# OPPO-Mente-Lab/PEA-Diffusion

Hardware: AMD Instinct MI355X
Metric: training images/sec (SDXL 1024px bf16, adapter-only bwd) (higher is better)
Workload: dtype bf16

## Files before the change

include/pea_hip.h:

```cpp
#ifndef PEA_HIP_H
#define PEA_HIP_H
#include <stdint.h>
#ifdef __cplusplus
extern "C" {
#endif

#define PEA_OK 0
#define PEA_E_INVALID (-1)
#define PEA_E_HIP (-2)
#define PEA_E_SHAPE (-3)
#define PEA_E_STATE (-4)
#define PEA_E_NOTFOUND (-5)
#define PEA_E_TIMEOUT (-6)

const char* pea_last_error(void);
int pea_version(void);
int pea_device_count(void);


int pea_op_gemm(const void* A, int lda, const void* W, int ldw, void* C, int ldc, int M, int N, int K, float alpha,
                const float* bias, const void* rowvec, int ldrv, int rows_per_batch, int act, void* preact,
                int ldpre, const void* res, int ldres, int out_f32, int accum_f32, void* stream);

int pea_op_gemm_qscale(const void* A, int lda, const void* W, int ldw, void* C, int ldc, int M, int N, int K, const float* bias,
                       int qscale_cols, float qscale, void* stream);

int pea_op_gemm_geglu(const void* A, int lda, const void* W, int ldw, const float* bias, void* y, void* stash, int M, int N,
                      int K, int stash_grad, int stash_rows, void* stream);

int pea_op_gemm_geglu_bwd(const void* A, int lda, const void* W, int ldw, const void* pre, int ldpre, void* C, int ldc,
                          int M, int N, int K, int form, void* stream);

int pea_op_ln_linear(const void* x, const float* gamma, const float* beta, const void* W, const float* bias, void* y,
                     void* geglu_y, int M, int N, int K, float eps, void* Wf, float* svec, float* tvec, float* stats,
                     void* stream);

int pea_op_conv3x3(const void* x, const void* w, void* y, int B, int Hs, int Ws, int Cin, int Cout, int stride,
                   int upsample2x, int transposed2, const float* bias, const void* rowvec, int ldrv,
                   const void* res, void* stream);
int pea_op_pack_conv(const float* w, void* out, int Co, int Ci, int dgrad, void* stream);
int pea_op_pack_conv_subpixel(const float* w, void* out, int Co, int Ci, int dgrad, void* stream);
int pea_op_concat2(const void* a, int C1, const void* b, int C2, void* y, long long rows, int aH, int aW, void* stream);
int pea_op_split2(const void* dy, int C1, int C2, void* da, int accum_a, void* db, int accum_b, long long rows, int aH,
                  int aW, void* stream);
long long pea_op_freeu_scratch_bytes(int B, int H, int W, int C2);
int pea_op_freeu_coef(const void* skip, int B, int H, int W, int C2, float* coef, void* scratch, void* stream);
int pea_op_concat2_freeu(const void* a, int C1, const void* b, int C2, const float* coef, void* y, int B, int H, int W, float s,
                         float bscale, int aH, int aW, void* stream);
int pea_op_upconv_subpixel(const void* x, const void* w, void* y, int B, int Hs, int Ws, int Cin, int Cout,
                           const float* bias, void* stream);
int pea_op_upconv_subpixel_dgrad(const void* dy, const void* wt, void* dx, int B, int Hs, int Ws, int Cin, int Cout,
                                 const void* res, void* stream);
int pea_op_conv_in(const float* x_nchw, const float* w, const float* bias, void* y_nhwc, int B, int Cin, int H,
                   int W, int Cout, void* stream);
int pea_op_conv_in_gather(const float* latents, const float* mask, const float* masked_latents, const float* w,
                          const float* bias, void* y_nhwc, int B, int C, int latent_batch, int cond_batch, int H, int W,
                          int Cout, void* stream);
int pea_op_conv_out(const void* x_nhwc, const float* w_packed, const float* bias, float* y_nchw, int B, int Cin,
                    int H, int W, int Cout, void* stream);
int pea_op_conv_out_dgrad(const float* dy_nchw, const float* w_packed, void* dx_nhwc, int B, int Cin, int H, int W,
                          int Cout, void* stream);
int pea_op_pack_conv_out(const float* w, float* out, int Co, int Ci, void* stream);

long long pea_op_groupnorm_scratch_bytes(int B, int HW, int C, int groups);
int pea_op_groupnorm_fwd(const void* x, const float* gamma, const float* beta, void* y, float* stats, void* scratch,
                         int B, int HW, int C, int groups, float eps, int silu, void* stream);
int pea_op_groupnorm_bwd(const void* x, const void* dy, const float* gamma, const float* beta, const float* stats,
                         void* dx, void* scratch, int B, int HW, int C, int groups, int silu, int accum,
                         void* stream);
int pea_op_layernorm_fwd(const void* x, const float* gamma, const float* beta, void* y, float* stats, int R, int C,
                         float eps, void* stream);
int pea_op_layernorm_fwd_f32(const float* x, const float* gamma, const float* beta, float* y, int R, int C, float eps,
                             void* stream);
int pea_op_layernorm_bwd(const void* x, const void* dy, const float* gamma, const float* stats, void* dx,
                         float* dgamma, float* dbeta, int R, int C, int accum, void* stream);

int pea_op_attention_fwd(const void* Q, int ldq, const void* K, int ldk, const void* V, int ldv, void* O, int ldo,
// ... 322 lines not shown
```

pea_diffusion_amd/csrc/api_ops.hip:

```cpp
#include <stdarg.h>
#include <string.h>

#include "../../include/pea_hip.h"
#include "pea_kernels.h"

static thread_local char g_err[512] = "";
void pea_set_error(const char* fmt, ...) {
  va_list ap;
  va_start(ap, fmt);
  vsnprintf(g_err, sizeof(g_err), fmt, ap);
  va_end(ap);
}

static bf16* g_zero_page = nullptr;
int pea_zero_page(const bf16** out) {
  if (!g_zero_page) {
    HIPCHK(hipMalloc((void**)&g_zero_page, 256));
    HIPCHK(hipMemset(g_zero_page, 0, 256));
  }
  *out = g_zero_page;
  return PEA_OK;
}

static AttnP attn_operands(const void* Q, int ldq, const void* K, int ldk, const void* V, int ldv, const void* O, int ldo,
// ... 25 lines not shown

extern "C" {

const char* pea_last_error(void) { return g_err; }
int pea_version(void) { return 100; }
int pea_device_count(void) {
  int n = 0;
  if (hipGetDeviceCount(&n) != hipSuccess) return 0;
  return n;
}

int pea_op_gemm(const void* A, int lda, const void* W, int ldw, void* C, int ldc, int M, int N, int K, float alpha,
                const float* bias, const void* rowvec, int ldrv, int rows_per_batch, int act, void* preact,
                int ldpre, const void* res, int ldres, int out_f32, int accum_f32, void* stream) {
  GemmP p;
  memset(&p, 0, sizeof(p));
  p.mode = 0;
  p.A = (const bf16*)A; p.lda = lda; p.W = (const bf16*)W; p.ldw = ldw; p.C = C; p.ldc = ldc;
  p.M = M; p.N = N; p.K = K; p.alpha = alpha; p.bias = bias;
  p.rowvec = (const bf16*)rowvec; p.ldrv = ldrv; p.rows_per_batch = rows_per_batch > 0 ? rows_per_batch : 1;
  p.act = act; p.preact = (bf16*)preact; p.ldpre = ldpre; p.res = (const bf16*)res; p.ldres = ldres;
  p.out_f32 = out_f32; p.accum_f32 = accum_f32;
  return launch_gemm(p, (hipStream_t)stream);
}

int pea_op_gemm_qscale(const void* A, int lda, const void* W, int ldw, void* C, int ldc, int M, int N, int K, const float* bias,
                       int qscale_cols, float qscale, void* stream) {
  GemmP p;
  memset(&p, 0, sizeof(p));
  p.A = (const bf16*)A; p.lda = lda; p.W = (const bf16*)W; p.ldw = ldw; p.C = C; p.ldc = ldc;
  p.M = M; p.N = N; p.K = K; p.alpha = 1.f; p.bias = bias; p.rows_per_batch = 1;
  p.qscale_cols = qscale_cols; p.qscale = qscale;
  return launch_gemm(p, (hipStream_t)stream);
}

int pea_op_gemm_geglu_bwd(const void* A, int lda, const void* W, int ldw, const void* pre, int ldpre, void* C, int ldc,
                          int M, int N, int K, int form, void* stream) {
  GemmP p;
  memset(&p, 0, sizeof(p));
  p.A = (const bf16*)A; p.lda = lda; p.W = (const bf16*)W; p.ldw = ldw; p.C = C; p.ldc = ldc;
  p.M = M; p.N = N; p.K = K; p.alpha = 1.f; p.rows_per_batch = 1;
  p.gbwd_pre = (const bf16*)pre; p.ldgp = ldpre; p.gbwd_form = form;
  return launch_gemm(p, (hipStream_t)stream);
}

int pea_op_gemm_geglu(const void* A, int lda, const void* W, int ldw, const float* bias, void* y, void* stash, int M, int N,
// ... 85 lines not shown
long long pea_op_freeu_scratch_bytes(int B, int H, int W, int C2) { return (long long)freeu_scratch_bytes(B, H, W, C2); }
int pea_op_freeu_coef(const void* skip, int B, int H, int W, int C2, float* coef, void* scratch, void* stream) {
  return launch_freeu_coef((const bf16*)skip, B, H, W, C2, coef, (float*)scratch, (hipStream_t)stream);
}
int pea_op_concat2_freeu(const void* a, int C1, const void* b, int C2, const float* coef, void* y, int B, int H, int W, float s,
                         float bscale, int aH, int aW, void* stream) {
  return launch_concat2_freeu((const bf16*)a, C1, (const bf16*)b, C2, coef, (bf16*)y, B, H, W, s, bscale, (hipStream_t)stream, aH, aW);
}
int pea_op_pack_conv_subpixel(const float* w, void* out, int Co, int Ci, int dgrad, void* stream) {
  return launch_pack_conv_subpix(w, (bf16*)out, Co, Ci, dgrad, (hipStream_t)stream);
}

int pea_op_pack_conv(const float* w, void* out, int Co, int Ci, int dgrad, void* stream) {
  return dgrad ? launch_pack_conv_dgrad(w, (bf16*)out, Co, Ci, (hipStream_t)stream)
               : launch_pack_conv_fwd(w, (bf16*)out, Co, Ci, (hipStream_t)stream);
}
int pea_op_pack_conv_out(const float* w, float* out, int Co, int Ci, void* stream) {
  return launch_pack_conv_out(w, out, Co, Ci, (hipStream_t)stream);
}
int pea_op_conv_in(const float* x, const float* w, const float* bias, void* y, int B, int Cin, int H, int W,
                   int Cout, void* stream) {
  return launch_conv_in(x, w, bias, (bf16*)y, B, Cin, H, W, Cout, (hipStream_t)stream);
}
int pea_op_conv_in_gather(const float* latents, const float* mask, const float* masked_latents, const float* w,
                          const float* bias, void* y, int B, int C, int latent_batch, int cond_batch, int H, int W, int Cout,
                          void* stream) {
  if (!w || !bias || !y) { pea_set_error("pea_op_conv_in_gather: null pointer"); return PEA_E_INVALID; }
  return launch_conv_in_gather(latents, mask, masked_latents, w, bias, (bf16*)y, B, C, latent_batch, cond_batch, H, W, Cout,
                               (hipStream_t)stream);
}
int pea_op_conv_out(const void* x, const float* w, const float* bias, float* y, int B, int Cin, int H, int W,
                    int Cout, void* stream) {
  return launch_conv_out((const bf16*)x, w, bias, y, B, Cin, H, W, Cout, (hipStream_t)stream);
}
int pea_op_conv_out_dgrad(const float* dy, const float* w, void* dx, int B, int Cin, int H, int W, int Cout,
                          void* stream) {
  return launch_conv_out_dgrad(dy, w, (bf16*)dx, B, Cin, H, W, Cout, (hipStream_t)stream);
}

int pea_op_groupnorm_fwd(const void* x, const float* gamma, const float* beta, void* y, float* stats, void* scratch,
                         int B, int HW, int C, int groups, float eps, int silu, void* stream) {
  return launch_groupnorm_fwd((const bf16*)x, gamma, beta, (bf16*)y, stats, (double*)scratch, B, HW, C, groups, eps,
                              silu, (hipStream_t)stream);
}
int pea_op_groupnorm_bwd(const void* x, const void* dy, const float* gamma, const float* beta, const float* stats,
                         void* dx, void* scratch, int B, int HW, int C, int groups, int silu, int accum,
// ... 247 lines not shown
```

pea_diffusion_amd/csrc/gemm.hip:

```cpp
#include <stdint.h>
#include <stdlib.h>

#include <type_traits>

#include "pea_kernels.h"

#define BK 64
constexpr int GEMM_ILV_M = 1;
constexpr int GEMM_ILV_HEAD = 4;

__device__ __forceinline__ int swz_off(int row, int chunk) { return row * 128 + ((chunk ^ ((row >> 1) & 7)) << 4); }

#ifdef PEA_GEMM_PROBES
#define PEA_PROBE(bit) (p.debug & (bit))
#else
#define PEA_PROBE(bit) false
#endif

template <int N>
__device__ __forceinline__ void wait_vmcnt() {
  static_assert(N >= 0 && N < 64, "vmcnt is a 6-bit counter");
  asm volatile("s_waitcnt vmcnt(%0)" ::"n"(N) : "memory");
}

// ... 1590 lines not shown
             "gemm: the folded-LayerNorm epilogue needs the batched-load epilogue (bf16 output, no activation / residual)");
  }
  int rc = PEA_OK;
  switch (d.inst) {
#define X(id, fn, cg, rf, gen, ...) \
    case GEMM_V##id: rc = p.mode == 0 ? fn<0, __VA_ARGS__>(p, stream) : fn<1, __VA_ARGS__>(p, stream); break;
    GEMM_TABLE(X)
#undef X
    case GEMM_GBWD_256: rc = launch_lcp<0, 256, 160, 4, 2, 4, 3, 0, 0, 3>(p, stream); break;
    case GEMM_GBWD_128: rc = launch_lcp<0, 128, 160, 4, 2, 4, 3, 0, 0, 3>(p, stream); break;
    case GEMM_GBWD_64: rc = launch_lcp<0, 64, 160, 2, 2, 4, 4, 0, 0, 3>(p, stream); break;
    case GEMM_LNF_256: rc = launch_lcp<0, 256, 160, 4, 2, 4, 3, 0, 0, 2>(p, stream); break;
    case GEMM_LNF_LC256: rc = launch_lc<0, 256, 160, 4, 2, 4, 3, false, true, 1, true>(p, stream); break;
    case GEMM_LNF_128: rc = launch_lcp<0, 128, 160, 4, 2, 4, 3, 0, 0, 2>(p, stream); break;
    case GEMM_LNF_64: rc = launch_lcp<0, 64, 160, 2, 2, 4, 4, 0, 0, 2>(p, stream); break;
    case GEMM_LNF_LC128: rc = launch_lc<0, 128, 160, 4, 2, 4, 3, false, true, 1, true>(p, stream); break;
  }
  PROF_END(stream);
  if (rc != PEA_OK) return rc;
  HIPCHK(hipGetLastError());
  return PEA_OK;
}

__global__ __launch_bounds__(256) void conv_in_kernel(const float* __restrict__ x, const float* __restrict__ w,
                                                      const float* __restrict__ bias, bf16* __restrict__ y, int B,
                                                      int Cin, int H, int W, int Cout, int pix_per_block, int ldy,
                                                      int silu) {
  extern __shared__ __attribute__((aligned(16))) char cism[];
  float* wl = (float*)cism;
  const int K = Cin * 9;
  for (int i = threadIdx.x; i < K * Cout; i += blockDim.x) {
    const int co = i / K, k = i - co * K;
    wl[k * Cout + co] = w[i];
  }
  __syncthreads();
  const int nchunk = Cout / 8;
  const int ppb = blockDim.x / nchunk;
  const int ck = threadIdx.x % nchunk, pl = threadIdx.x / nchunk;
  if (pl >= ppb) return;
  const int c0 = ck * 8;
  float bs[8];
#pragma unroll
  for (int j = 0; j < 8; ++j) bs[j] = bias[c0 + j];
  const long long npix = (long long)B * H * W;
  const long long p0 = (long long)blockIdx.x * pix_per_block;
  const long long p1 = p0 + pix_per_block < npix ? p0 + pix_per_block : npix;
// ... 11 lines not shown
          const int ix = xw + kx - 1;
          const bool ok = (unsigned)iy < (unsigned)H && (unsigned)ix < (unsigned)W;
          const float v = ok ? x[(((long long)b * Cin + ci) * H + iy) * W + ix] : 0.f;
          const float* wr = wl + (ci * 9 + ky * 3 + kx) * Cout + c0;
          const f32x4 w0 = *(const f32x4*)wr, w1 = *(const f32x4*)(wr + 4);
#pragma unroll
          for (int j = 0; j < 4; ++j) {
            acc[j] += v * w0[j];
            acc[4 + j] += v * w1[j];
          }
        }
      }
    bf16x8 o;
#pragma unroll
    for (int j = 0; j < 8; ++j) o[j] = (bf16)(silu ? siluf_(acc[j]) : acc[j]);
    *(bf16x8*)(y + pix * ldy + c0) = o;
  }
}

struct ConvGatherSrc {
  const float* lat; const float* mask; const float* masked;
  int C, lat_b, cond_b;
};
template <bool FLIP, bool GATHER = false>
__global__ __launch_bounds__(256) void conv_few4_kernel(const float* __restrict__ x, const float* __restrict__ w,
                                                        const float* __restrict__ bias, bf16* __restrict__ y, int B,
                                                        int Cs, int H, int W, int N, int groups_per_block, int ldy,
                                                        int silu, ConvGatherSrc gs) {
  extern __shared__ __attribute__((aligned(16))) char cfsm[];
  float* wl = (float*)cfsm;
  const int K = Cs * 9;
  for (int i = threadIdx.x; i < K * N; i += blockDim.x) {
    if (FLIP) {
      wl[i] = w[i];
    } else {
      const int n = i / K, k = i - n * K;
      wl[k * N + n] = w[i];
    }
  }
  __syncthreads();
  const int nchunk = N / 8;
  const int ppb = blockDim.x / nchunk;
  const int ck = threadIdx.x % nchunk, pl = threadIdx.x / nchunk;
  if (pl >= ppb) return;
  const int c0 = ck * 8;
  float bs[8];
#pragma unroll
  for (int j = 0; j < 8; ++j) bs[j] = bias ? bias[c0 + j] : 0.f;
  const int W4 = W / 4;
  const long long ngroups = (long long)B * H * W4;
  const long long g0 = (long long)blockIdx.x * groups_per_block;
  const long long g1 = g0 + groups_per_block < ngroups ? g0 + groups_per_block : ngroups;
  for (long long grp = g0 + pl; grp < g1; grp += ppb) {
    const int x0 = (int)(grp % W4) * 4, yh = (int)((grp / W4) % H), b = (int)(grp / ((long long)W4 * H));
    float acc[4][8];
#pragma unroll
    for (int p = 0; p < 4; ++p)
#pragma unroll
      for (int j = 0; j < 8; ++j) acc[p][j] = bs[j];
    const long long HW = (long long)H * W;
    const int bl = GATHER ? b % gs.lat_b : 0, bc = GATHER ? b % gs.cond_b : 0;
    for (int ci = 0; ci < Cs; ++ci)
#pragma unroll
      for (int ky = 0; ky < 3; ++ky) {
        const int iy = FLIP ? yh + 1 - ky : yh + ky - 1;
        if ((unsigned)iy >= (unsigned)H) continue;
        const float* row;
        if constexpr (GATHER) {
          const float* plane = ci < gs.C    ? gs.lat + ((long long)bl * gs.C + ci) * HW
                               : ci == gs.C ? gs.mask + (long long)bc * HW
                                            : gs.masked + ((long long)bc * (Cs - gs.C - 1) + (ci - gs.C - 1)) * HW;
          row = plane + (long long)iy * W;
        } else {
          row = x + (((long long)b * Cs + ci) * H + iy) * W;
        }
        float v[6];
        const f32x4 mid = *(const f32x4*)(row + x0);
        v[0] = x0 > 0 ? row[x0 - 1] : 0.f;
        v[1] = mid[0]; v[2] = mid[1]; v[3] = mid[2]; v[4] = mid[3];
        v[5] = x0 + 4 < W ? row[x0 + 4] : 0.f;
#pragma unroll
        for (int kx = 0; kx < 3; ++kx) {
          const float* wr = wl + (ci * 9 + ky * 3 + kx) * N + c0;
          const f32x4 w0 = *(const f32x4*)wr, w1 = *(const f32x4*)(wr + 4);
#pragma unroll
          for (int p = 0; p < 4; ++p) {
            const float vv = FLIP ? v[p + 2 - kx] : v[p + kx];
#pragma unroll
            for (int j = 0; j < 4; ++j) {
              acc[p][j] += vv * w0[j];
              acc[p][4 + j] += vv * w1[j];
            }
          }
        }
      }
    const long long pix = ((long long)b * H + yh) * W + x0;
#pragma unroll
    for (int p = 0; p < 4; ++p) {
      bf16x8 o;
#pragma unroll
      for (int j = 0; j < 8; ++j) o[j] = (bf16)(silu ? siluf_(acc[p][j]) : acc[p][j]);
      *(bf16x8*)(y + (pix + p) * ldy + c0) = o;
    }
  }
}

template <bool FLIP, bool GATHER = false>
static bool launch_conv_few4(const float* x, const float* w, const float* bias, bf16* y, int B, int Cs, int H, int W, int N,
                             int ldy, int silu, hipStream_t s, int* rc, const ConvGatherSrc& gs = ConvGatherSrc{}) {
  const size_t lds = (size_t)Cs * 9 * N * 4;
  if (!GATHER && (W % 4 != 0 || N % 8 != 0 || N / 8 > 256 || lds > 160 * 1024 || (((unsigned long long)x) & 15) != 0))
    return false;
  *rc = PEA_OK;
  if (lds > 64 * 1024) {
    static bool attr_set = false;
    if (!attr_set) {
      if (hipFuncSetAttribute((const void*)conv_few4_kernel<FLIP, GATHER>, hipFuncAttributeMaxDynamicSharedMemorySize, 160 * 1024) != hipSuccess) {
        *rc = PEA_E_HIP;
        return true;
      }
      attr_set = true;
    }
  }
  const int ppb = 256 / (N / 8);
  const long long ngroups = (long long)B * H * (W / 4);
  long long per = cdivl(ngroups, 768);
  per = cdivl(per, ppb) * ppb;
  hipLaunchKernelGGL((conv_few4_kernel<FLIP, GATHER>), dim3((unsigned)cdivl(ngroups, per)), dim3(256), lds, s, x, w, bias, y, B, Cs,
                     H, W, N, (int)per, ldy, silu, gs);
  if (hipGetLastError() != hipSuccess) *rc = PEA_E_HIP;
  return true;
}

int launch_conv_in(const float* x, const float* w, const float* bias, bf16* y, int B, int Cin, int H, int W,
                   int Cout, hipStream_t s, int ldy, int silu) {
  if (ldy <= 0) ldy = Cout;
  {
    int rc;
    if (launch_conv_few4<false>(x, w, bias, y, B, Cin, H, W, Cout, ldy, silu, s, &rc)) return rc;
  }
  SHAPECHK(Cout % 8 == 0 && Cout / 8 <= 256 && Cin * 9 * Cout * 4 <= 160 * 1024, "conv_in: Cout=%d Cin=%d", Cout, Cin);
  if (Cin * 9 * Cout * 4 > 64 * 1024) {
    static bool attr_set = false;
    if (!attr_set) {
      HIPCHK(hipFuncSetAttribute((const void*)conv_in_kernel, hipFuncAttributeMaxDynamicSharedMemorySize, 160 * 1024));
      attr_set = true;
    }
  }
  const int nchunk = Cout / 8;
  const int ppb = 256 / nchunk;
  const int per = ppb * 8;
  const long long npix = (long long)B * H * W;
  hipLaunchKernelGGL(conv_in_kernel, dim3((unsigned)cdivl(npix, per)), dim3(256), (size_t)Cin * 9 * Cout * 4, s, x, w,
                     bias, y, B, Cin, H, W, Cout, per, ldy, silu);
  HIPCHK(hipGetLastError());
  return PEA_OK;
}

int launch_conv_in_gather(const float* lat, const float* mask, const float* masked, const float* w, const float* bias, bf16* y,
                          int B, int C, int lat_b, int cond_b, int H, int W, int Cout, hipStream_t s, int ldy) {
  if (ldy <= 0) ldy = Cout;
  const int Cs = 2 * C + 1;
  auto al16 = [](const float* p) { return p != nullptr && (((unsigned long long)p) & 15) == 0; };
  SHAPECHK(C > 0 && lat_b > 0 && cond_b > 0 && B % lat_b == 0 && B % cond_b == 0,
           "conv_in_gather: B=%d must be a multiple of latent_batch=%d and cond_batch=%d", B, lat_b, cond_b);
  SHAPECHK(W % 4 == 0 && Cout % 8 == 0 && Cout / 8 <= 256 && (size_t)Cs * 9 * Cout * 4 <= 160 * 1024,
           "conv_in_gather: W=%d must be a multiple of 4, Cout=%d of 8 (%d input channels)", W, Cout, Cs);
  SHAPECHK(al16(lat) && al16(mask) && al16(masked), "conv_in_gather: latents / mask / masked latents must be 16-byte aligned");
  int rc = PEA_OK;
  launch_conv_few4<false, true>(nullptr, w, bias, y, B, Cs, H, W, Cout, ldy, 0, s, &rc,
                                ConvGatherSrc{lat, mask, masked, C, lat_b, cond_b});
  if (rc != PEA_OK) pea_set_error("conv_in_gather: launch failed");
  return rc;
}

__global__ __launch_bounds__(256) void conv_out_kernel(const bf16* __restrict__ x, const float* __restrict__ w,
                                                       const float* __restrict__ bias, float* __restrict__ y,
                                                       int B, int Cin, int H, int W, int Cout) {
  const int lane = threadIdx.x & 63;
  const long long pix = (long long)blockIdx.x * 4 + (threadIdx.x >> 6);
  if (pix >= (long long)B * H * W) return;
  const int xw = (int)(pix % W), yh = (int)((pix / W) % H), b = (int)(pix / ((long long)W * H));
  float acc[8] = {0.f, 0.f, 0.f, 0.f, 0.f, 0.f, 0.f, 0.f};
  const int cchunks = Cin / 8;
  for (int i = lane; i < 9 * cchunks; i += 64) {
    const int tap = i / cchunks, c8 = (i - tap * cchunks) * 8;
    const int ky = tap / 3, kx = tap - ky * 3;
    const int iy = yh + ky - 1, ix = xw + kx - 1;
    if ((unsigned)iy >= (unsigned)H || (unsigned)ix >= (unsigned)W) continue;
    const bf16x8 v = *(const bf16x8*)(x + (((long long)b * H + iy) * W + ix) * Cin + c8);
#pragma unroll
    for (int co = 0; co < 8; ++co) {
      if (co < Cout) {
        const float* wp = w + ((long long)co * 9 + tap) * Cin + c8;
// ... 135 lines not shown
  for (int co = 0; co < Cout; ++co)
    for (int ky = 0; ky < 3; ++ky) {
      const int oy = yh + 1 - ky;
      if ((unsigned)oy >= (unsigned)H) continue;
      for (int kx = 0; kx < 3; ++kx) {
        const int ox = xw + 1 - kx;
        if ((unsigned)ox >= (unsigned)W) continue;
        const float g = dy[(((long long)b * Cout + co) * H + oy) * W + ox];
        const float* wp = w + ((long long)co * 9 + ky * 3 + kx) * Cin + c8;
#pragma unroll
        for (int j = 0; j < 8; ++j) acc[j] += g * wp[j];
      }
    }
  bf16x8 o;
#pragma unroll
  for (int j = 0; j < 8; ++j) o[j] = (bf16)acc[j];
  *(bf16x8*)(dx + pix * Cin + c8) = o;
}

int launch_conv_out_dgrad(const float* dy, const float* w, bf16* dx, int B, int Cin, int H, int W, int Cout,
                          hipStream_t s) {
  {
    int rc;
    if (launch_conv_few4<true>(dy, w, nullptr, dx, B, Cout, H, W, Cin, Cin, 0, s, &rc)) return rc;
  }
  const long long total = (long long)B * H * W * (Cin / 8);
  hipLaunchKernelGGL(conv_out_dgrad_kernel, dim3((unsigned)cdivl(total, 256)), dim3(256), 0, s, dy, w, dx, B, Cin,
                     H, W, Cout);
  HIPCHK(hipGetLastError());
  return PEA_OK;
}

__global__ void splitk_reduce_kernel(const float* __restrict__ part, int nsplit, long long stride, bf16* __restrict__ out,
                                     int ldo, int M, int N, int accum) {
  const long long total = (long long)M * (N / 4);
  for (long long i = (long long)blockIdx.x * blockDim.x + threadIdx.x; i < total;
       i += (long long)gridDim.x * blockDim.x) {
    const int m = (int)(i / (N / 4)), n = (int)(i % (N / 4)) * 4;
    f32x4 a = {0.f, 0.f, 0.f, 0.f};
    for (int s = 0; s < nsplit; ++s) {
      const f32x4 v = *(const f32x4*)(part + s * stride + (long long)m * N + n);
#pragma unroll
      for (int j = 0; j < 4; ++j) a[j] += v[j];
    }
    bf16* dst = out + (long long)m * ldo + n;
    bf16x4 o;
    if (accum) o = *(const bf16x4*)dst;
// ... 14 lines not shown
```

pea_diffusion_amd/csrc/pea_kernels.h:

```cpp
#pragma once
#include "pea_common.h"

struct GemmP {
  int mode;
  const bf16* A; int lda;
  const bf16* W; int ldw;
  void* C; int ldc; int out_f32;
  int accum_f32;
  int M, N, K;
  float alpha;
  const float* bias;
  const bf16* rowvec; int ldrv; int rows_per_batch;
  int act;
  bf16* preact; int ldpre;
  const bf16* res; int ldres;
  int Hs, Ws, Cin, Ho, Wo;
  int stride;
  int pad_off;
  int shift;
  int parity;
  int kside;
  int pad_dx;
  int pix;
  const bf16* zeros;
  int debug;
  bf16* geglu_y; int ldy;
  int geglu_tanh;
  int stash_rows;
  int stash_grad;
  int ksplit; long long split_stride;
  int epi_fast;
  const float* ln_stats; const float* ln_s;
  const bf16* gbwd_pre; int ldgp;
  int qscale_cols; float qscale;
  int gbwd_form;
  const void* pf_ptr; long long pf_bytes;
};
int launch_splitk_reduce(const float* part, int nsplit, long long stride, bf16* out, int ldo, int M, int N, int accum,
                         hipStream_t s);
int launch_gemm(const GemmP& p, hipStream_t stream);

int launch_conv_in(const float* x, const float* w, const float* bias, bf16* y, int B, int Cin, int H, int W,
                   int Cout, hipStream_t s, int ldy = 0, int silu = 0);
int launch_conv_in_gather(const float* lat, const float* mask, const float* masked, const float* w, const float* bias, bf16* y,
                          int B, int C, int lat_b, int cond_b, int H, int W, int Cout, hipStream_t s, int ldy = 0);
int launch_conv_out(const bf16* x, const float* w, const float* bias, float* y, int B, int Cin, int H, int W,
                    int Cout, hipStream_t s);
int launch_conv_out_dgrad(const float* dy, const float* w, bf16* dx, int B, int Cin, int H, int W, int Cout,
                          hipStream_t s);

int launch_groupnorm_fwd(const bf16* x, const float* gamma, const float* beta, bf16* y, float* stats,
                         double* scratch, int B, int HW, int C, int groups, float eps, int silu, hipStream_t s);
int launch_groupnorm_bwd(const bf16* x, const bf16* dy, const float* gamma, const float* beta, const float* stats,
                         bf16* dx, double* scratch, int B, int HW, int C, int groups, int silu, const bf16* add,
                         hipStream_t s);
int launch_layernorm_fwd(const bf16* x, const float* gamma, const float* beta, bf16* y, float* stats, int R, int C,
                         float eps, hipStream_t s);
int launch_rmsnorm_fwd(const bf16* x, const float* gamma, bf16* y, int R, int C, float eps, hipStream_t s);
int launch_layernorm_fwd_f32(const float* x, const float* gamma, const float* beta, float* y, int R, int C, float eps,
                             hipStream_t s);
int launch_layernorm_stats(const bf16* x, float* stats, int R, int C, float eps, hipStream_t s);
int launch_ln_fold(const bf16* W, int ldw, const float* gamma, const float* beta, const float* bias, bf16* Wf, float* svec,
                   float* tvec, int N, int K, hipStream_t s);
// ... 199 lines not shown
```

pea_diffusion_amd/csrc/tape.hip:

```cpp
#include <stdlib.h>

#include <algorithm>

#include "model.h"

int Tape::alloc() {
  tag_q_prescale();
  for (const Op& o : ops) {
    const int in[5] = {o.a, o.kind == OP_LINEAR || o.kind == OP_EMBED ? -1 : o.b, o.kind == OP_LINEAR || o.kind == OP_EMBED ? -1 : o.c, o.res, o.rv};
    for (int k = 0; k < 5; ++k) {
      if (in[k] < 0 || in[k] >= (int)tn.size() || !tn[in[k]].d2s) continue;
      SHAPECHK(o.kind == OP_CONCAT && k == 0 && o.a != o.b, "tape: op kind %d reads a depth-to-space tensor", o.kind);
    }
  }
  size_t off = 0;
  size_t max_numel = 0;
  if (owns_weights) {
    for (FusedMat& f : fused) {
      f.off_w = off; off += al256((size_t)f.N * f.K * 2);
      if (f.need_wt) { f.off_wt = off; off += al256((size_t)f.N * f.K * 2); }
      if (f.has_bias) { f.off_bias = off; off += al256((size_t)f.N * 4); }
    }
    for (WSlot& s : slots) {
      max_numel = std::max(max_numel, (size_t)s.numel);
// ... 598 lines not shown
  RC(rc_ops);
  if (graph == 2) ce_valid = true;
  return PEA_OK;
}

int Tape::gemm(GemmP& p, hipStream_t s) {
  if (WSeq* q = wseq_cur) {
    const long long bytes = (p.ldw == p.K && p.ksplit <= 1) ? (long long)p.N * p.K * 2 : 0;
    if (!q->ready) q->w.push_back({(const void*)p.W, bytes});
    else {
      const size_t i = q->pos++;
      if (i >= q->w.size() || q->w[i].first != (const void*)p.W) { q->ready = false; q->w.clear(); wseq_cur = nullptr; }
      else {
        if (i + 1 < q->w.size()) {
          const Tape* ow = weights_owner ? weights_owner : this;
          const char* t = (const char*)q->w[i + 1].first;
          const long long nb = q->w[i + 1].second;
          if (ow->warena && t >= ow->warena && t + nb <= ow->warena + ow->wbytes) { p.pf_ptr = t; p.pf_bytes = nb; }
          else { q->ready = false; q->w.clear(); wseq_cur = nullptr; }
        }
      }
    }
  }
  return launch_gemm(p, s);
}

int Tape::exec_ops(size_t begin, size_t end, bool skip_cached, hipStream_t s) {
  RC(ensure_acts());
  for (size_t oi = begin; oi < end; ++oi) {
    Op& o = ops[oi];
    if (skip_cached && ce_valid && (int)oi >= ce_begin && (int)oi < ce_end) continue;
    switch (o.kind) {
      case OP_TEMB: {
        Tn& out = tn[o.out];
        if (o.src == 0) RC(launch_timestep_embed(t_in, out.d, B, o.p0, s));
        else RC(launch_timestep_embed(tid_in, out.d, B * 6, o.p0, s));
        break;
      }
      case OP_LINEAR: {
        Tn &a = tn[o.a], &out = tn[o.out];
        GemmP p; fill_gemm(p);
        p.A = a.d; p.lda = a.cols; p.M = (int)a.rows; p.K = a.cols; p.N = out.cols;
        if (o.fused >= 0) { FusedMat& f = fused[o.fused]; p.W = f.w; p.ldw = f.K; p.bias = f.bias; }
        else { WSlot& w = slots[o.w]; p.W = w.w; p.ldw = w.ldw; p.bias = o.bias >= 0 ? slots[o.bias].f32 : nullptr; }
        p.C = out.d; p.ldc = out.cols; p.act = o.p2;
        p.qscale_cols = o.qs_cols; p.qscale = o.qs;
        if (o.p3 == 3) {
// ... 437 lines not shown
```

pea_diffusion_amd/ops.py:

```python
from __future__ import annotations

import ctypes
from typing import List, Optional, Sequence

import torch

from ._lib import PeaError, check, lib, ptr, stream_ptr

BF = torch.bfloat16


def _dev(t):
    return t.device


def gemm(a, w, bias=None, rowvec=None, rows_per_batch=1, act=0, res=None, want_preact=False, out_f32=False,
         alpha=1.0, out=None, accum_f32=False):
    M, K = a.shape
    N = w.shape[0]
    if out is None:
        out = torch.empty(M, N, device=a.device, dtype=torch.float32 if out_f32 else BF)
    pre = torch.empty(M, N, device=a.device, dtype=BF) if want_preact else None
    check(lib().pea_op_gemm(ptr(a), a.stride(0), ptr(w), w.stride(0), ptr(out), out.stride(0), M, N, K, alpha,
                            ptr(bias), ptr(rowvec), rowvec.stride(0) if rowvec is not None else 0, rows_per_batch,
                            act, ptr(pre), N, ptr(res), res.stride(0) if res is not None else 0,
                            int(out.dtype == torch.float32), int(accum_f32), stream_ptr()))
    return (out, pre) if want_preact else out


def gemm_geglu(a, w, bias=None, want_stash=True, stash_grad=True, stash_rows=0):
    M, K = a.shape
    N = w.shape[0]
    y = torch.empty(M, N // 2, device=a.device, dtype=BF)
    st = torch.zeros(M, N, device=a.device, dtype=BF) if want_stash else None
    check(lib().pea_op_gemm_geglu(ptr(a), a.stride(0), ptr(w), w.stride(0), ptr(bias), ptr(y), ptr(st), M, N, K,
                                  int(stash_grad), stash_rows, stream_ptr()))
    return y, st


def gemm_geglu_bwd(a, w, pre, form=0):
    M, K = a.shape
    N = w.shape[0]
    out = torch.empty(M, 2 * N, device=a.device, dtype=BF)
    check(lib().pea_op_gemm_geglu_bwd(ptr(a), a.stride(0), ptr(w), w.stride(0), ptr(pre), pre.stride(0), ptr(out), out.stride(0),
                                      M, N, K, form, stream_ptr()))
    return out


def ln_linear(x, gamma, beta, w, bias=None, eps=1e-5, geglu=False):
# ... 86 lines not shown
            coef = torch.empty(B, 7, C2, device=b.device, dtype=torch.float32)
        nbytes = freeu_scratch_bytes(B, H, W, C2)
        if scratch is None and nbytes:
            scratch = torch.empty(nbytes // 4, device=b.device, dtype=torch.float32)
        check(lib().pea_op_freeu_coef(ptr(b), B, H, W, C2, ptr(coef), ptr(scratch), stream_ptr()))
    else:
        coef = None
    check(lib().pea_op_concat2_freeu(ptr(a), C1, ptr(b), C2, ptr(coef), ptr(y), B, H, W, float(s), float(bscale),
                                     H if d2s else 0, W if d2s else 0, stream_ptr()))
    return y, coef


def split2(dy, C1, C2, da=None, db=None, accum_a=False, accum_b=False, d2s_hw=None):
    rows = dy.numel() // (C1 + C2)
    H, W = d2s_hw if d2s_hw else (0, 0)
    check(lib().pea_op_split2(ptr(dy), C1, C2, ptr(da), int(accum_a), ptr(db), int(accum_b), rows, H, W, stream_ptr()))


def conv_in(x_nchw, w, bias):
    B, Cin, H, W = x_nchw.shape
    Cout = w.shape[0]
    y = torch.empty(B, H, W, Cout, device=x_nchw.device, dtype=BF)
    check(lib().pea_op_conv_in(ptr(x_nchw), ptr(w.contiguous()), ptr(bias), ptr(y), B, Cin, H, W, Cout, stream_ptr()))
    return y


def conv_in_gather(latents, mask, masked_latents, w, bias, B):
    lb, C, H, W = latents.shape
    cb = mask.shape[0]
    Cout = w.shape[0]
    y = torch.empty(B, H, W, Cout, device=latents.device, dtype=BF)
    check(lib().pea_op_conv_in_gather(ptr(latents), ptr(mask), ptr(masked_latents), ptr(w.contiguous()), ptr(bias), ptr(y), B,
                                      C, lb, cb, H, W, Cout, stream_ptr()))
    return y


def inpaint_prepare(image, mask):
    N, _, H, W = image.shape
    init = torch.empty_like(image)
    masked = torch.empty_like(image)
    lmask = torch.empty(N, 1, H // 8, W // 8, device=image.device, dtype=torch.float32)
    check(lib().pea_op_inpaint_prepare(ptr(image), ptr(mask), N, H, W, ptr(init), ptr(masked), ptr(lmask), stream_ptr()))
    return init, masked, lmask


def pack_conv_out(w):
# ... 415 lines not shown
```

Measured before the change: 41.60.

## Add skinny-M split-K MFMA GEMM and MFMA-based few-channel conv kernel

Adds a dedicated kernel for GEMMs with at most 16 rows. It spreads the K dimension across up to 16 waves, each using 16x16x32 bf16 MFMA, and reduces the partial sums through LDS. The tape linear path now routes through it, falling back to the generic GEMM when the shape or alignment checks fail. Separately, the scalar FMA conv_few4 kernel used by conv_in, conv_in_gather and the conv_out dgrad is replaced by an f32 MFMA (16x16x4) kernel that keeps the weights pre-swizzled in LDS. This aims to cut latency on small-M linears such as the timestep and text embeddings and on the first and last convolutions. The cost is new code paths with extra shape and alignment constraints, and a different accumulation order.

```diff
diff --git a/include/pea_hip.h b/include/pea_hip.h
--- a/include/pea_hip.h
+++ b/include/pea_hip.h
@@ -21,6 +21,10 @@
 int pea_op_gemm(const void* A, int lda, const void* W, int ldw, void* C, int ldc, int M, int N, int K, float alpha,
                 const float* bias, const void* rowvec, int ldrv, int rows_per_batch, int act, void* preact,
                 int ldpre, const void* res, int ldres, int out_f32, int accum_f32, void* stream);
+
+int pea_op_gemm_rows(const void* A, int lda, const void* W, int ldw, void* C, int ldc, int M, int N, int K, float alpha,
+                     const float* bias, const void* rowvec, int ldrv, int rows_per_batch, int act, void* preact,
+                     int ldpre, const void* res, int ldres, int out_f32, int accum_f32, void* stream);
 
 int pea_op_gemm_qscale(const void* A, int lda, const void* W, int ldw, void* C, int ldc, int M, int N, int K, const float* bias,
                        int qscale_cols, float qscale, void* stream);
@@ -53,6 +57,8 @@
                                  const void* res, void* stream);
 int pea_op_conv_in(const float* x_nchw, const float* w, const float* bias, void* y_nhwc, int B, int Cin, int H,
                    int W, int Cout, void* stream);
+int pea_op_conv_in_strided(const float* x_nchw, const float* w, const float* bias, void* y_nhwc, int B, int Cin, int H,
+                           int W, int Cout, int ldy, int silu, void* stream);
 int pea_op_conv_in_gather(const float* latents, const float* mask, const float* masked_latents, const float* w,
                           const float* bias, void* y_nhwc, int B, int C, int latent_batch, int cond_batch, int H, int W,
                           int Cout, void* stream);
diff --git a/pea_diffusion_amd/csrc/api_ops.hip b/pea_diffusion_amd/csrc/api_ops.hip
--- a/pea_diffusion_amd/csrc/api_ops.hip
+++ b/pea_diffusion_amd/csrc/api_ops.hip
@@ -71,6 +71,20 @@
   p.act = act; p.preact = (bf16*)preact; p.ldpre = ldpre; p.res = (const bf16*)res; p.ldres = ldres;
   p.out_f32 = out_f32; p.accum_f32 = accum_f32;
   return launch_gemm(p, (hipStream_t)stream);
+}
+
+int pea_op_gemm_rows(const void* A, int lda, const void* W, int ldw, void* C, int ldc, int M, int N, int K, float alpha,
+                     const float* bias, const void* rowvec, int ldrv, int rows_per_batch, int act, void* preact,
+                     int ldpre, const void* res, int ldres, int out_f32, int accum_f32, void* stream) {
+  GemmP p;
+  memset(&p, 0, sizeof(p));
+  p.mode = 0;
+  p.A = (const bf16*)A; p.lda = lda; p.W = (const bf16*)W; p.ldw = ldw; p.C = C; p.ldc = ldc;
+  p.M = M; p.N = N; p.K = K; p.alpha = alpha; p.bias = bias;
+  p.rowvec = (const bf16*)rowvec; p.ldrv = ldrv; p.rows_per_batch = rows_per_batch > 0 ? rows_per_batch : 1;
+  p.act = act; p.preact = (bf16*)preact; p.ldpre = ldpre; p.res = (const bf16*)res; p.ldres = ldres;
+  p.out_f32 = out_f32; p.accum_f32 = accum_f32;
+  return launch_gemm_rows(p, (hipStream_t)stream);
 }
 
 int pea_op_gemm_qscale(const void* A, int lda, const void* W, int ldw, void* C, int ldc, int M, int N, int K, const float* bias,
@@ -202,6 +216,10 @@
                    int Cout, void* stream) {
   return launch_conv_in(x, w, bias, (bf16*)y, B, Cin, H, W, Cout, (hipStream_t)stream);
 }
+int pea_op_conv_in_strided(const float* x, const float* w, const float* bias, void* y, int B, int Cin, int H, int W,
+                           int Cout, int ldy, int silu, void* stream) {
+  return launch_conv_in(x, w, bias, (bf16*)y, B, Cin, H, W, Cout, (hipStream_t)stream, ldy, silu);
+}
 int pea_op_conv_in_gather(const float* latents, const float* mask, const float* masked_latents, const float* w,
                           const float* bias, void* y, int B, int C, int latent_batch, int cond_batch, int H, int W, int Cout,
                           void* stream) {
diff --git a/pea_diffusion_amd/csrc/gemm.hip b/pea_diffusion_amd/csrc/gemm.hip
--- a/pea_diffusion_amd/csrc/gemm.hip
+++ b/pea_diffusion_amd/csrc/gemm.hip
@@ -1636,6 +1636,80 @@
   return PEA_OK;
 }
 
+constexpr int ROWS_MAX_WAVES = 16;
+static int gemm_rows_waves(int K) {
+  const int nsteps = K / BK;
+  return nsteps < 8 ? 4 : (nsteps < 64 ? 8 : ROWS_MAX_WAVES);
+}
+__global__ __launch_bounds__(ROWS_MAX_WAVES * 64) void gemm_rows_kernel(const GemmP p) {
+  __shared__ f32x4 part[ROWS_MAX_WAVES][64];
+  const int lane = threadIdx.x & 63, w = threadIdx.x >> 6, nw = blockDim.x >> 6;
+  const int r16 = lane & 15, q4 = lane >> 4;
+  const int n0 = blockIdx.x * 16;
+  const int nsteps = p.K / BK;
+  const bool live = r16 < p.M;
+  const bf16* wp = p.W + (long long)min(n0 + r16, p.N - 1) * p.ldw + q4 * 16;
+  const bf16* ap = p.A + (long long)(live ? r16 : 0) * p.lda + q4 * 16;
+  f32x4 acc[1][1];
+  acc[0][0] = (f32x4){0.f, 0.f, 0.f, 0.f};
+  for (int s0 = w; s0 < nsteps; s0 += 4 * nw) {
+    bf16x8 wf[4][2], af[4][2];
+#pragma unroll
+    for (int u = 0; u < 4; ++u) {
+#pragma unroll
+      for (int h = 0; h < 2; ++h)
+#pragma unroll
+        for (int j = 0; j < 8; ++j) { wf[u][h][j] = (bf16)0.f; af[u][h][j] = (bf16)0.f; }
+      const int s = s0 + u * nw;
+      if (s < nsteps) {
+        wf[u][0] = *(const bf16x8*)(wp + (long long)s * BK);
+        wf[u][1] = *(const bf16x8*)(wp + (long long)s * BK + 8);
+        if (live) {
+          af[u][0] = *(const bf16x8*)(ap + (long long)s * BK);
+          af[u][1] = *(const bf16x8*)(ap + (long long)s * BK + 8);
+        }
+      }
+    }
+#pragma unroll
+    for (int u = 0; u < 4; ++u) {
+      if (s0 + u * nw < nsteps) {
+        acc[0][0] = __builtin_amdgcn_mfma_f32_16x16x32_bf16(wf[u][0], af[u][0], acc[0][0], 0, 0, 0);
+        acc[0][0] = __builtin_amdgcn_mfma_f32_16x16x32_bf16(wf[u][1], af[u][1], acc[0][0], 0, 0, 0);
+      }
+    }
+  }
+  dma_prefetch_next(p, blockIdx.x * nw + w, gridDim.x * nw, lane);
+  part[w][lane] = acc[0][0];
+  __syncthreads();
+  if (w != 0) return;
+  for (int i = 1; i < nw; ++i) acc[0][0] += part[i][lane];
+  gemm_epilogue16<1, 1>(p, acc, 0, n0, r16, q4);
+}
+
+static bool gemm_rows_takes(const GemmP& p) {
+  auto al = [](const void* q, int b) { return ((unsigned long long)q & (unsigned long long)(b - 1)) == 0; };
+  return g_gemm_variant < 0 && p.mode == 0 && p.M >= 1 && p.M <= 16 && p.N > 0 && p.N % 4 == 0 && p.K > 0 && p.K % BK == 0 &&
+         p.ldw == p.K && p.lda % 8 == 0 && p.ldc % 4 == 0 && p.A && p.W && p.C && al(p.A, 16) && al(p.W, 16) &&
+         al(p.C, p.out_f32 ? 16 : 8) && (long long)p.N * p.K * 2 <= 0x7fffffffLL && !p.accum_f32 && !p.rowvec && !p.geglu_y &&
+         !p.gbwd_pre && !p.ln_stats && !p.qscale_cols && p.ksplit <= 1 && (p.act == 0 || p.act == 2) &&
+         (!p.bias || al(p.bias, 16)) && (!p.preact || (al(p.preact, 8) && p.ldpre % 4 == 0)) &&
+         (!p.res || (al(p.res, 8) && p.ldres % 4 == 0));
+}
+
+int launch_gemm_rows(const GemmP& p_in, hipStream_t stream) {
+  if (!gemm_rows_takes(p_in)) return launch_gemm(p_in, stream);
+  GemmP p = p_in;
+  if (g_prof_on) { g_prof_tag[0] = p.M; g_prof_tag[1] = p.N; g_prof_tag[2] = p.K; g_prof_tag[3] = (p.res ? 1 : 0) | (p.bias ? 2 : 0); }
+  PROF_BEGIN(0, 2.0 * p.M * (double)p.N * p.K, 2.0 * ((double)p.M * p.N + (double)p.N * p.K + (double)p.M * p.K), stream);
+  const GemmEnv& env = gemm_env();
+  if (!env.pf_on || p.pf_bytes <= 0) { p.pf_ptr = nullptr; p.pf_bytes = 0; }
+  if (p.pf_bytes > env.pf_max) p.pf_bytes = env.pf_max;
+  hipLaunchKernelGGL(gemm_rows_kernel, dim3(cdiv(p.N, 16)), dim3(gemm_rows_waves(p.K) * 64), 0, stream, p);
+  PROF_END(stream);
+  HIPCHK(hipGetLastError());
+  return PEA_OK;
+}
+
 __global__ __launch_bounds__(256) void conv_in_kernel(const float* __restrict__ x, const float* __restrict__ w,
                                                       const float* __restrict__ bias, bf16* __restrict__ y, int B,
                                                       int Cin, int H, int W, int Cout, int pix_per_block, int ldy,
@@ -1693,112 +1767,140 @@
   const float* lat; const float* mask; const float* masked;
   int C, lat_b, cond_b;
 };
-template <bool FLIP, bool GATHER = false>
-__global__ __launch_bounds__(256) void conv_few4_kernel(const float* __restrict__ x, const float* __restrict__ w,
-                                                        const float* __restrict__ bias, bf16* __restrict__ y, int B,
-                                                        int Cs, int H, int W, int N, int groups_per_block, int ldy,
-                                                        int silu, ConvGatherSrc gs) {
+constexpr int CONV_FEW_KSMAX = 21;
+template <bool FLIP, bool GATHER, int NP>
+__global__ __launch_bounds__(512) void conv_few_mfma_kernel(const float* __restrict__ x, const float* __restrict__ w,
+                                                            const float* __restrict__ bias, bf16* __restrict__ y, int B,
+                                                            int Cs, int H, int W, int N, int tiles_per_block, int ldy,
+                                                            int silu, ConvGatherSrc gs) {
   extern __shared__ __attribute__((aligned(16))) char cfsm[];
   float* wl = (float*)cfsm;
-  const int K = Cs * 9;
-  for (int i = threadIdx.x; i < K * N; i += blockDim.x) {
-    if (FLIP) {
-      wl[i] = w[i];
-    } else {
-      const int n = i / K, k = i - n * K;
-      wl[k * N + n] = w[i];
-    }
-  }
+  constexpr int TPL = 2 * NP;
+  const int K = Cs * 9, ks3 = (K + 11) / 12 * 3;
+  const int nchunks = (N + 32 * NP - 1) / (32 * NP);
+  for (int i = threadIdx.x; i < ks3 * nchunks * 64 * TPL; i += blockDim.x) wl[i] = 0.f;
   __syncthreads();
-  const int nchunk = N / 8;
-  const int ppb = blockDim.x / nchunk;
-  const int ck = threadIdx.x % nchunk, pl = threadIdx.x / nchunk;
-  if (pl >= ppb) return;
-  const int c0 = ck * 8;
-  float bs[8];
-#pragma unroll
-  for (int j = 0; j < 8; ++j) bs[j] = bias ? bias[c0 + j] : 0.f;
-  const int W4 = W / 4;
-  const long long ngroups = (long long)B * H * W4;
-  const long long g0 = (long long)blockIdx.x * groups_per_block;
-  const long long g1 = g0 + groups_per_block < ngroups ? g0 + groups_per_block : ngroups;
-  for (long long grp = g0 + pl; grp < g1; grp += ppb) {
-    const int x0 = (int)(grp % W4) * 4, yh = (int)((grp / W4) % H), b = (int)(grp / ((long long)W4 * H));
-    float acc[4][8];
-#pragma unroll
-    for (int p = 0; p < 4; ++p)
-#pragma unroll
-      for (int j = 0; j < 8; ++j) acc[p][j] = bs[j];
-    const long long HW = (long long)H * W;
+  for (int i0 = threadIdx.x; i0 < N * K; i0 += 8 * blockDim.x) {
+    float v[8];
+#pragma unroll
+    for (int e = 0; e < 8; ++e) {
+      const int i = i0 + e * blockDim.x;
+      v[e] = i < N * K ? w[i] : 0.f;
+    }
+#pragma unroll
+    for (int e = 0; e < 8; ++e) {
+      const int i = i0 + e * blockDim.x;
+      const int n = FLIP ? i % N : i / K, k = FLIP ? i / N : i - n * K;
+      const int t = (n >> 5) * 2 + ((n >> 2) & 1), r = ((n >> 3) & 3) * 4 + (n & 3);
+      if (i < N * K) wl[((((k >> 2) * nchunks + t / TPL) * 64) + (k & 3) * 16 + r) * TPL + t % TPL] = v[e];
+    }
+  }
+  __syncthreads();
+  const int lane = threadIdx.x & 63, wv = threadIdx.x >> 6;
+  const int pl = lane & 15, q = lane >> 4;
+  const int HW = H * W, npix = B * HW;
+  const int ntile = (npix + 15) / 16;
+  const int t0 = blockIdx.x * tiles_per_block;
+  const int t1 = t0 + tiles_per_block < ntile ? t0 + tiles_per_block : ntile;
+  int kt[CONV_FEW_KSMAX];
+#pragma unroll
+  for (int s = 0; s < CONV_FEW_KSMAX; ++s) {
+    const int k = 4 * s + q, ci = k / 9, r = k - 9 * ci, ky = r / 3, kx = r - 3 * ky;
+    kt[s] = k < K ? (ci | (FLIP ? 2 - ky : ky) << 8 | (FLIP ? 2 - kx : kx) << 12) : -1;
+  }
+  for (int tile = t0 + wv; tile < t1; tile += (int)(blockDim.x >> 6)) {
+    const int pix = tile * 16 + pl;
+    const bool pok = pix < npix;
+    const int pc = pok ? pix : npix - 1;
+    const int b = pc / HW, rem = pc - b * HW, yh = rem / W, xw = rem - yh * W;
     const int bl = GATHER ? b % gs.lat_b : 0, bc = GATHER ? b % gs.cond_b : 0;
-    for (int ci = 0; ci < Cs; ++ci)
-#pragma unroll
-      for (int ky = 0; ky < 3; ++ky) {
-        const int iy = FLIP ? yh + 1 - ky : yh + ky - 1;
-        if ((unsigned)iy >= (unsigned)H) continue;
-        const float* row;
+    float bv[CONV_FEW_KSMAX];
+#pragma unroll
+    for (int s = 0; s < CONV_FEW_KSMAX; ++s) {
+      bv[s] = 0.f;
+      const int e = kt[s];
+      const int ci = e & 255, iy = yh + ((e >> 8) & 15) - 1, ix = xw + ((e >> 12) & 15) - 1;
+      if (pok && e >= 0 && (unsigned)iy < (unsigned)H && (unsigned)ix < (unsigned)W) {
+        const float* plane;
         if constexpr (GATHER) {
-          const float* plane = ci < gs.C    ? gs.lat + ((long long)bl * gs.C + ci) * HW
-                               : ci == gs.C ? gs.mask + (long long)bc * HW
-                                            : gs.masked + ((long long)bc * (Cs - gs.C - 1) + (ci - gs.C - 1)) * HW;
-          row = plane + (long long)iy * W;
+          plane = ci < gs.C    ? gs.lat + ((long long)bl * gs.C + ci) * HW
+                  : ci == gs.C ? gs.mask + (long long)bc * HW
+                               : gs.masked + ((long long)bc * (Cs - gs.C - 1) + (ci - gs.C - 1)) * HW;
         } else {
-          row = x + (((long long)b * Cs + ci) * H + iy) * W;
-        }
-        float v[6];
-        const f32x4 mid = *(const f32x4*)(row + x0);
-        v[0] = x0 > 0 ? row[x0 - 1] : 0.f;
-        v[1] = mid[0]; v[2] = mid[1]; v[3] = mid[2]; v[4] = mid[3];
-        v[5] = x0 + 4 < W ? row[x0 + 4] : 0.f;
-#pragma unroll
-        for (int kx = 0; kx < 3; ++kx) {
-          const float* wr = wl + (ci * 9 + ky * 3 + kx) * N + c0;
-          const f32x4 w0 = *(const f32x4*)wr, w1 = *(const f32x4*)(wr + 4);
-#pragma unroll
-          for (int p = 0; p < 4; ++p) {
-            const float vv = FLIP ? v[p + 2 - kx] : v[p + kx];
-#pragma unroll
-            for (int j = 0; j < 4; ++j) {
-              acc[p][j] += vv * w0[j];
-              acc[p][4 + j] += vv * w1[j];
-            }
-          }
-        }
-      }
-    const long long pix = ((long long)b * H + yh) * W + x0;
-#pragma unroll
-    for (int p = 0; p < 4; ++p) {
-      bf16x8 o;
-#pragma unroll
-      for (int j = 0; j < 8; ++j) o[j] = (bf16)(silu ? siluf_(acc[p][j]) : acc[p][j]);
-      *(bf16x8*)(y + (pix + p) * ldy + c0) = o;
+          plane = x + ((long long)b * Cs + ci) * HW;
+        }
+        bv[s] = plane[iy * W + ix];
+      }
+    }
+    for (int chunk = 0; chunk < nchunks; ++chunk) {
+      f32x4 bq[NP][2];
+#pragma unroll
+      for (int u = 0; u < NP; ++u) {
+        const int n = (chunk * NP + u) * 32 + 8 * q;
+        bq[u][0] = bq[u][1] = (f32x4){0.f, 0.f, 0.f, 0.f};
+        if (bias && n < N) { bq[u][0] = *(const f32x4*)(bias + n); bq[u][1] = *(const f32x4*)(bias + n + 4); }
+      }
+      f32x4 acc[TPL];
+#pragma unroll
+      for (int t = 0; t < TPL; ++t) acc[t] = (f32x4){0.f, 0.f, 0.f, 0.f};
+      const float* wa = wl + (chunk * 64 + lane) * TPL;
+#pragma unroll
+      for (int sb = 0; sb < CONV_FEW_KSMAX; sb += 3) {
+        if (sb < ks3) {
+          float af[3][TPL];
+#pragma unroll
+          for (int d = 0; d < 3; ++d)
+#pragma unroll
+            for (int t = 0; t < TPL; ++t) af[d][t] = wa[(sb + d) * nchunks * 64 * TPL + t];
+#pragma unroll
+          for (int d = 0; d < 3; ++d)
+#pragma unroll
+            for (int t = 0; t < TPL; ++t) acc[t] = __builtin_amdgcn_mfma_f32_16x16x4f32(af[d][t], bv[sb + d], acc[t], 0, 0, 0);
+        }
+      }
+#pragma unroll
+      for (int u = 0; u < NP; ++u) {
+        const int n = (chunk * NP + u) * 32 + 8 * q;
+        bf16x8 o;
+#pragma unroll
+        for (int j = 0; j < 8; ++j) {
+          const float v = acc[2 * u + (j >> 2)][j & 3] + bq[u][j >> 2][j & 3];
+          o[j] = (bf16)(silu ? siluf_(v) : v);
+        }
+        if (pok && n < N) *(bf16x8*)(y + (long long)pix * ldy + n) = o;
+      }
     }
   }
 }
 
 template <bool FLIP, bool GATHER = false>
-static bool launch_conv_few4(const float* x, const float* w, const float* bias, bf16* y, int B, int Cs, int H, int W, int N,
-                             int ldy, int silu, hipStream_t s, int* rc, const ConvGatherSrc& gs = ConvGatherSrc{}) {
-  const size_t lds = (size_t)Cs * 9 * N * 4;
-  if (!GATHER && (W % 4 != 0 || N % 8 != 0 || N / 8 > 256 || lds > 160 * 1024 || (((unsigned long long)x) & 15) != 0))
+static bool launch_conv_few_mfma(const float* x, const float* w, const float* bias, bf16* y, int B, int Cs, int H, int W, int N,
+                                 int ldy, int silu, hipStream_t s, int* rc, const ConvGatherSrc& gs = ConvGatherSrc{}) {
+  const int NP = N % 64 == 0 ? 2 : 1;
+  const int ks3 = (Cs * 9 + 11) / 12 * 3, ntiles = cdiv(N, 32 * NP) * NP * 2;
+  const size_t lds = (size_t)ks3 * ntiles * 64 * 4;
+  if (N % 8 != 0 || ldy % 8 != 0 || (((unsigned long long)y) & 15) != 0 || (((unsigned long long)bias) & 15) != 0 ||
+      ks3 > CONV_FEW_KSMAX || lds > 160 * 1024 || (long long)B * H * W > 0x7fffffffLL - 16)
     return false;
   *rc = PEA_OK;
+  const void* fn = NP == 2 ? (const void*)conv_few_mfma_kernel<FLIP, GATHER, 2> : (const void*)conv_few_mfma_kernel<FLIP, GATHER, 1>;
   if (lds > 64 * 1024) {
-    static bool attr_set = false;
-    if (!attr_set) {
-      if (hipFuncSetAttribute((const void*)conv_few4_kernel<FLIP, GATHER>, hipFuncAttributeMaxDynamicSharedMemorySize, 160 * 1024) != hipSuccess) {
+    static bool attr_set[2] = {false, false};
+    if (!attr_set[NP - 1]) {
+      if (hipFuncSetAttribute(fn, hipFuncAttributeMaxDynamicSharedMemorySize, 160 * 1024) != hipSuccess) {
         *rc = PEA_E_HIP;
         return true;
       }
-      attr_set = true;
-    }
-  }
-  const int ppb = 256 / (N / 8);
-  const long long ngroups = (long long)B * H * (W / 4);
-  long long per = cdivl(ngroups, 768);
-  per = cdivl(per, ppb) * ppb;
-  hipLaunchKernelGGL((conv_few4_kernel<FLIP, GATHER>), dim3((unsigned)cdivl(ngroups, per)), dim3(256), lds, s, x, w, bias, y, B, Cs,
-                     H, W, N, (int)per, ldy, silu, gs);
+      attr_set[NP - 1] = true;
+    }
+  }
+  const long long ntile = cdivl((long long)B * H * W, 16);
+  const long long per = cdivl(cdivl(ntile, 512), 8) * 8;
+  const dim3 grid((unsigned)cdivl(ntile, per));
+  if (NP == 2)
+    hipLaunchKernelGGL((conv_few_mfma_kernel<FLIP, GATHER, 2>), grid, dim3(512), lds, s, x, w, bias, y, B, Cs, H, W, N, (int)per, ldy, silu, gs);
+  else
+    hipLaunchKernelGGL((conv_few_mfma_kernel<FLIP, GATHER, 1>), grid, dim3(512), lds, s, x, w, bias, y, B, Cs, H, W, N, (int)per, ldy, silu, gs);
   if (hipGetLastError() != hipSuccess) *rc = PEA_E_HIP;
   return true;
 }
@@ -1808,7 +1910,7 @@
   if (ldy <= 0) ldy = Cout;
   {
     int rc;
-    if (launch_conv_few4<false>(x, w, bias, y, B, Cin, H, W, Cout, ldy, silu, s, &rc)) return rc;
+    if (launch_conv_few_mfma<false>(x, w, bias, y, B, Cin, H, W, Cout, ldy, silu, s, &rc)) return rc;
   }
   SHAPECHK(Cout % 8 == 0 && Cout / 8 <= 256 && Cin * 9 * Cout * 4 <= 160 * 1024, "conv_in: Cout=%d Cin=%d", Cout, Cin);
   if (Cin * 9 * Cout * 4 > 64 * 1024) {
@@ -1839,8 +1941,9 @@
            "conv_in_gather: W=%d must be a multiple of 4, Cout=%d of 8 (%d input channels)", W, Cout, Cs);
   SHAPECHK(al16(lat) && al16(mask) && al16(masked), "conv_in_gather: latents / mask / masked latents must be 16-byte aligned");
   int rc = PEA_OK;
-  launch_conv_few4<false, true>(nullptr, w, bias, y, B, Cs, H, W, Cout, ldy, 0, s, &rc,
-                                ConvGatherSrc{lat, mask, masked, C, lat_b, cond_b});
+  const bool taken = launch_conv_few_mfma<false, true>(nullptr, w, bias, y, B, Cs, H, W, Cout, ldy, 0, s, &rc,
+                                                       ConvGatherSrc{lat, mask, masked, C, lat_b, cond_b});
+  SHAPECHK(taken, "conv_in_gather: output row stride %d must be a multiple of 8 and y 16-byte aligned", ldy);
   if (rc != PEA_OK) pea_set_error("conv_in_gather: launch failed");
   return rc;
 }
@@ -2022,7 +2125,7 @@
                           hipStream_t s) {
   {
     int rc;
-    if (launch_conv_few4<true>(dy, w, nullptr, dx, B, Cout, H, W, Cin, Cin, 0, s, &rc)) return rc;
+    if (launch_conv_few_mfma<true>(dy, w, nullptr, dx, B, Cout, H, W, Cin, Cin, 0, s, &rc)) return rc;
   }
   const long long total = (long long)B * H * W * (Cin / 8);
   hipLaunchKernelGGL(conv_out_dgrad_kernel, dim3((unsigned)cdivl(total, 256)), dim3(256), 0, s, dy, w, dx, B, Cin,
diff --git a/pea_diffusion_amd/csrc/pea_kernels.h b/pea_diffusion_amd/csrc/pea_kernels.h
--- a/pea_diffusion_amd/csrc/pea_kernels.h
+++ b/pea_diffusion_amd/csrc/pea_kernels.h
@@ -39,6 +39,7 @@
 int launch_splitk_reduce(const float* part, int nsplit, long long stride, bf16* out, int ldo, int M, int N, int accum,
                          hipStream_t s);
 int launch_gemm(const GemmP& p, hipStream_t stream);
+int launch_gemm_rows(const GemmP& p, hipStream_t stream);
 
 int launch_conv_in(const float* x, const float* w, const float* bias, bf16* y, int B, int Cin, int H, int W,
                    int Cout, hipStream_t s, int ldy = 0, int silu = 0);
diff --git a/pea_diffusion_amd/csrc/tape.hip b/pea_diffusion_amd/csrc/tape.hip
--- a/pea_diffusion_amd/csrc/tape.hip
+++ b/pea_diffusion_amd/csrc/tape.hip
@@ -644,7 +644,7 @@
       }
     }
   }
-  return launch_gemm(p, s);
+  return launch_gemm_rows(p, s);
 }
 
 int Tape::exec_ops(size_t begin, size_t end, bool skip_cached, hipStream_t s) {
diff --git a/pea_diffusion_amd/ops.py b/pea_diffusion_amd/ops.py
--- a/pea_diffusion_amd/ops.py
+++ b/pea_diffusion_amd/ops.py
@@ -25,6 +25,20 @@
                             ptr(bias), ptr(rowvec), rowvec.stride(0) if rowvec is not None else 0, rows_per_batch,
                             act, ptr(pre), N, ptr(res), res.stride(0) if res is not None else 0,
                             int(out.dtype == torch.float32), int(accum_f32), stream_ptr()))
+    return (out, pre) if want_preact else out
+
+
+def gemm_rows(a, w, bias=None, rowvec=None, rows_per_batch=1, act=0, res=None, want_preact=False, out_f32=False,
+              alpha=1.0, out=None, accum_f32=False):
+    M, K = a.shape
+    N = w.shape[0]
+    if out is None:
+        out = torch.empty(M, N, device=a.device, dtype=torch.float32 if out_f32 else BF)
+    pre = torch.empty(M, N, device=a.device, dtype=BF) if want_preact else None
+    check(lib().pea_op_gemm_rows(ptr(a), a.stride(0), ptr(w), w.stride(0), ptr(out), out.stride(0), M, N, K, alpha,
+                                 ptr(bias), ptr(rowvec), rowvec.stride(0) if rowvec is not None else 0, rows_per_batch,
+                                 act, ptr(pre), N, ptr(res), res.stride(0) if res is not None else 0,
+                                 int(out.dtype == torch.float32), int(accum_f32), stream_ptr()))
     return (out, pre) if want_preact else out
 
 
@@ -157,6 +171,15 @@
     Cout = w.shape[0]
     y = torch.empty(B, H, W, Cout, device=x_nchw.device, dtype=BF)
     check(lib().pea_op_conv_in(ptr(x_nchw), ptr(w.contiguous()), ptr(bias), ptr(y), B, Cin, H, W, Cout, stream_ptr()))
+    return y
+
+
+def conv_in_strided(x_nchw, w, bias, ldy, silu=False):
+    B, Cin, H, W = x_nchw.shape
+    Cout = w.shape[0]
+    y = torch.zeros(B, H, W, ldy, device=x_nchw.device, dtype=BF)
+    check(lib().pea_op_conv_in_strided(ptr(x_nchw), ptr(w.contiguous()), ptr(bias), ptr(y), B, Cin, H, W, Cout, ldy, int(silu),
+                                       stream_ptr()))
     return y
 
 
```

New measurement: 41.76 (median of 6 runs). No clear change (+0.4%).
